# TritonDataCenter/containerpilot

Hardware: AMD Instinct MI355X
Metric: events/sec (higher is better)
Workload: dtype n/a (CPU daemon, no tensor math; see BASELINE.json north_star); 1 GPU; model=containerpilot daemon, BASELINE stress shape scaled to 550 jobs, jobs=550, watches=50, parallelism=1 independent daemons (1/rank)

## Files before the change

### containerpilot_amd/native.py

```python

import ctypes
import json
import os

from . import REPO_ROOT

_LIB_PATH = os.path.join(REPO_ROOT, "containerpilot_amd", "_native.so")
_lib = None


def _load():
    global _lib
    if _lib is None:
        if not os.path.exists(_LIB_PATH):
            raise RuntimeError(
                "native library missing: %s (run __graft_entry__.build())"
                % _LIB_PATH)
        _lib = ctypes.CDLL(_LIB_PATH)
        _lib.cp_version.restype = ctypes.c_char_p
        _lib.cp_render_template.restype = ctypes.c_void_p
        _lib.cp_render_template.argtypes = [
            ctypes.c_char_p, ctypes.POINTER(ctypes.c_void_p)]
        _lib.cp_parse_duration_ns.restype = ctypes.c_longlong
        _lib.cp_parse_duration_ns.argtypes = [ctypes.c_char_p]
# ... 11 lines not shown
        _lib.cp_validate_config.argtypes = [ctypes.c_char_p]
        _lib.cp_consul_endpoint.restype = ctypes.c_void_p
        _lib.cp_consul_endpoint.argtypes = [
            ctypes.c_char_p, ctypes.POINTER(ctypes.c_void_p)]
        _lib.cp_watch_render.restype = ctypes.c_void_p
        _lib.cp_watch_render.argtypes = [
            ctypes.c_char_p, ctypes.c_char_p, ctypes.c_char_p,
            ctypes.c_char_p, ctypes.c_char_p,
            ctypes.POINTER(ctypes.c_void_p)]
        _lib.cp_kv_decode.restype = ctypes.c_void_p
        _lib.cp_kv_decode.argtypes = [
            ctypes.c_char_p, ctypes.c_size_t,
            ctypes.POINTER(ctypes.c_void_p)]
        _lib.cp_kv_render.restype = ctypes.c_void_p
        _lib.cp_kv_render.argtypes = [
            ctypes.c_char_p, ctypes.c_char_p, ctypes.c_size_t,
            ctypes.c_char_p, ctypes.c_char_p, ctypes.c_int,
            ctypes.c_char_p, ctypes.POINTER(ctypes.c_size_t),
            ctypes.POINTER(ctypes.c_void_p)]
        _lib.cp_sensor_extract.restype = ctypes.c_int
        _lib.cp_sensor_extract.argtypes = [
            ctypes.c_char_p, ctypes.c_size_t, ctypes.c_char_p,
            ctypes.POINTER(ctypes.c_double),
            ctypes.POINTER(ctypes.c_void_p)]
        _lib.cp_signal_number.restype = ctypes.c_int
        _lib.cp_signal_number.argtypes = [
            ctypes.c_char_p, ctypes.POINTER(ctypes.c_void_p)]
        _lib.cp_metrics_replay.restype = ctypes.c_void_p
        _lib.cp_metrics_replay.argtypes = [
            ctypes.c_char_p, ctypes.POINTER(ctypes.c_void_p)]
        _lib.cp_metric_value_string.restype = ctypes.c_void_p
        _lib.cp_metric_value_string.argtypes = [
            ctypes.c_char_p, ctypes.POINTER(ctypes.c_void_p)]
        _lib.cp_free.argtypes = [ctypes.c_void_p]
    return _lib


def _take_string(lib, ptr):
    if not ptr:
        return None
    out = ctypes.string_at(ptr).decode()
    lib.cp_free(ptr)
    return out


def version():
    return _load().cp_version().decode()


def render_template(text):
    lib = _load()
    err = ctypes.c_void_p()
    out = lib.cp_render_template(text.encode(), ctypes.byref(err))
    if not out:
        raise ValueError(_take_string(lib, err.value))
    return _take_string(lib, out)


def parse_duration_ns(text):
    ns = _load().cp_parse_duration_ns(text.encode())
    if ns < 0:
        raise ValueError("invalid duration: %s" % text)
    return ns


def parse_duration(text):
# ... 77 lines not shown
    err = ctypes.c_void_p()
    out = lib.cp_kv_decode(body, len(body), ctypes.byref(err))
    if not out:
        raise ValueError(_take_string(lib, err.value))
    return json.loads(_take_string(lib, out))


def kv_render(template_text, body, name, key, prefix=False, dc=""):
    lib = _load()
    if isinstance(body, str):
        body = body.encode()
    err = ctypes.c_void_p()
    size = ctypes.c_size_t()
    out = lib.cp_kv_render(template_text.encode(), body,
                           len(body) if body is not None else 0,
                           name.encode(), key.encode(), int(bool(prefix)),
                           dc.encode(), ctypes.byref(size), ctypes.byref(err))
    if not out:
        raise ValueError(_take_string(lib, err.value))
    rendered = ctypes.string_at(out, size.value)
    lib.cp_free(out)
    return rendered


def metrics_replay(script_json):
    lib = _load()
    err = ctypes.c_void_p()
    out = lib.cp_metrics_replay(script_json.encode(), ctypes.byref(err))
    if not out:
        raise ValueError(_take_string(lib, err.value))
    return _take_string(lib, out)


def metric_value_string(json_text):
    lib = _load()
    err = ctypes.c_void_p()
    out = lib.cp_metric_value_string(json_text.encode(), ctypes.byref(err))
    if not out:
        raise ValueError(_take_string(lib, err.value))
    return _take_string(lib, out)
```

### cpp/include/cpilot/command.hpp

```cpp
#pragma once

#include <memory>
#include <string>
#include <vector>

#include "cpilot/events.hpp"
#include "cpilot/json.hpp"
#include "cpilot/loop.hpp"
#include "cpilot/timing.hpp"

namespace cpilot {

bool parseArgs(const Json& raw, std::string* exec,
               std::vector<std::string>* args, std::string* err);

class Command : public std::enable_shared_from_this<Command> {
 public:
  Command(std::string execPath, std::vector<std::string> args, Duration timeout,
          bool raw, std::string logField);
  Command(const Command&) = delete;
  Command& operator=(const Command&) = delete;

  const std::string& name() const { return name_; }
  void setName(std::string name) { name_ = std::move(name); }
  const std::string& execPath() const { return exec_; }

  std::string envName() const;

  void run(Loop& loop, std::shared_ptr<Bus> bus);

  void term();
  void kill();

  bool running() const { return running_; }
  pid_t pid() const { return pid_; }

 private:
  void spawn(Loop& loop, std::shared_ptr<Bus> bus);
  void onExit(Loop& loop, std::shared_ptr<Bus> bus, int status);

  std::string name_;
  std::string exec_;
  std::vector<std::string> args_;
  Duration timeout_;
  bool raw_;
  std::string logField_;
  std::string pidEnvName_;

  pid_t pid_ = -1;
  bool running_ = false;
  bool pendingRun_ = false;
  int pendingSignal_ = 0;
  Loop* loop_ = nullptr;
  uint64_t timeoutTimer_ = 0;
  TimePoint tReq_{}, tCb_{};
  int logFd_ = -1;
  std::string logBuf_;
};

using CommandPtr = std::shared_ptr<Command>;

void commandEnvInvalidate();

CommandPtr newCommand(const Json& rawExec, Duration timeout, bool raw,
                      const std::string& logField, std::string* err);

}
```

### cpp/include/cpilot/spawner.hpp

```cpp
#pragma once

#include <sys/types.h>

#include <cstdint>
#include <deque>
#include <functional>
#include <map>
#include <memory>
#include <mutex>
#include <string>
#include <thread>
#include <vector>

#include "cpilot/loop.hpp"

namespace cpilot {

class Spawner {
 public:
  using SpawnCb = std::function<void(pid_t pid, int err)>;

  static Spawner& global();

  void spawn(Loop& loop, const std::string& execPath,
             const std::vector<std::string>& args,
             std::shared_ptr<const std::vector<std::string>> baseEnv,
             const std::vector<std::string>& extraEnv, int stdioFd,
             SpawnCb cb);

  int helperCount() const { return (int)helpers_.size(); }

  size_t backlog();
  bool overloaded();

 private:
  Spawner();
  struct Helper {
    int sock = -1;
    pid_t pid = -1;
    bool dead = false;
    std::deque<std::pair<std::vector<char>, int>> overflow;
    std::mutex sendMu;
  };
  struct Pending {
    Loop* loop;
    uint64_t loopId;
    SpawnCb cb;
    size_t helperIdx;
  };

  bool launchHelper(Helper* h);
  void flushOverflow(size_t idx);
  void readerMain();
  void handleMessage(size_t idx, const char* buf, size_t len);
  void helperDied(size_t idx);
  bool sendRequest(Helper& h, const std::vector<char>& buf, int fd);
  void wakeReader();

  std::string helperPath_;
  std::vector<std::unique_ptr<Helper>> helpers_;
  size_t nextHelper_ = 0;

  std::mutex mu_;
  std::map<uint32_t, Pending> pending_;
  uint32_t nextReqId_ = 1;
  std::map<pid_t, std::pair<Loop*, uint64_t>> pidLoops_;

  int wakeFds_[2] = {-1, -1};
  std::thread reader_;
};

}
```

### cpp/include/cpilot/spawnproto.hpp

```cpp
#pragma once

#include <cstdint>

namespace cpilot {
namespace spawnproto {

constexpr int kHelperFd = 3;

enum MsgType : uint32_t {
  kSpawnRequest = 1,
  kSpawnReply = 2,
  kChildExit = 3,
};

struct RequestHeader {
  uint32_t type;
  uint32_t reqId;
  uint32_t argc;
  uint32_t envc;
  uint8_t wantStdio;
  uint8_t pad[3];
};

struct Reply {
  uint32_t type;
  uint32_t reqId;
  int32_t pid;
  int32_t err;
};

struct ExitNotice {
  uint32_t type;
  uint32_t pad;
  int32_t pid;
  int32_t status;
};

constexpr size_t kMaxRequestBytes = 1024 * 1024;

}
}
```

### cpp/src/command.cpp

```cpp
#include "cpilot/command.hpp"

#include <fcntl.h>
#include <signal.h>
#include <sys/epoll.h>
#include <sys/wait.h>
#include <unistd.h>

#include <cctype>
#include <cstring>
#include <cstdio>
#include <map>

#include "cpilot/log.hpp"
#include "cpilot/spawner.hpp"

extern char** environ;

namespace cpilot {

namespace {

std::map<std::string, std::string>& pidEnvOverlay() {
  static std::map<std::string, std::string> overlay;
  return overlay;
}

std::shared_ptr<const std::vector<std::string>>& baseEnvCache() {
  static std::shared_ptr<const std::vector<std::string>> cache;
  return cache;
}
bool& baseEnvDirty() {
  static bool dirty = true;
  return dirty;
}

std::shared_ptr<const std::vector<std::string>> baseEnvSnapshot() {
  if (!baseEnvDirty() && baseEnvCache()) return baseEnvCache();
// ... 20 lines not shown

const std::vector<std::string>& overlayExtras() { return overlayStrings(); }

void overlaySet(const std::string& key, const std::string& value) {
  auto [it, inserted] = pidEnvOverlay().emplace(key, value);
  if (inserted) {
    overlayIndex()[key] = overlayStrings().size();
    overlayStrings().push_back(key + "=" + value);
    if (getenv(key.c_str())) baseEnvDirty() = true;
  } else {
    it->second = value;
    overlayStrings()[overlayIndex()[key]] = key + "=" + value;
  }
}

void overlayErase(const std::string& key) {
  if (pidEnvOverlay().erase(key)) {
    auto idxIt = overlayIndex().find(key);
    if (idxIt != overlayIndex().end()) {
      size_t slot = idxIt->second;
      overlayIndex().erase(idxIt);
      auto& strs = overlayStrings();
      if (slot + 1 != strs.size()) {
        strs[slot] = std::move(strs.back());
        size_t eq = strs[slot].find('=');
        overlayIndex()[strs[slot].substr(0, eq)] = slot;
      }
      strs.pop_back();
    }
    if (getenv(key.c_str())) baseEnvDirty() = true;
  }
}

}

void commandEnvInvalidate() { baseEnvDirty() = true; }

bool parseArgs(const Json& raw, std::string* execPath,
               std::vector<std::string>* args, std::string* err) {
  std::vector<std::string> all;
  if (raw.isString()) {
    std::string s = raw.str();
    size_t a = 0, b = s.size();
    while (a < b && isspace((unsigned char)s[a])) a++;
    while (b > a && isspace((unsigned char)s[b - 1])) b--;
    s = s.substr(a, b - a);
    if (!s.empty()) {
      std::string cur;
      for (char c : s) {
        if (c == ' ') {
          all.push_back(cur);
          cur.clear();
        } else {
          cur += c;
        }
      }
      all.push_back(cur);
    }
  } else if (raw.isArray()) {
    for (auto& e : raw.array()) {
      if (e.isString()) all.push_back(e.str());
      else all.push_back(e.dump());
    }
  } else if (!raw.isNull()) {
    *err = "unable to parse exec arguments";
    return false;
  }
  if (all.empty()) {
    *err = "received zero-length argument";
// ... 8 lines not shown
                      const std::string& logField, std::string* err) {
  std::string execPath;
  std::vector<std::string> args;
  if (!parseArgs(rawExec, &execPath, &args, err)) return nullptr;
  return std::make_shared<Command>(execPath, args, timeout, raw, logField);
}

Command::Command(std::string execPath, std::vector<std::string> args,
                 Duration timeout, bool raw, std::string logField)
    : name_(execPath),
      exec_(std::move(execPath)),
      args_(std::move(args)),
      timeout_(timeout),
      raw_(raw),
      logField_(std::move(logField)) {}

std::string Command::envName() const {
  if (name_.empty()) return name_;
  std::string name = name_;
  size_t slash = name.find_last_of('/');
  if (slash != std::string::npos) name = name.substr(slash + 1);
  size_t dot = name.find_last_of('.');
  if (dot != std::string::npos && dot > 0)
    name = name.substr(0, dot) + name.substr(name.size());
  std::string out;
  for (char c : name) {
    if (isalnum((unsigned char)c)) {
      out += (char)toupper((unsigned char)c);
    } else if (out.empty() || out.back() != '_') {
      out += '_';
    }
  }
  return out;
}

void Command::run(Loop& loop, std::shared_ptr<Bus> bus) {
  if (running_) {
    LOG_DEBUG("%s already running, queueing run", name_.c_str());
    pendingRun_ = true;
    return;
  }
  spawn(loop, std::move(bus));
}

void Command::spawn(Loop& loop, std::shared_ptr<Bus> bus) {
  loop_ = &loop;
  LOG_DEBUG("%s.Run start", name_.c_str());

  int pipefds[2] = {-1, -1};
  if (!raw_) {
    if (pipe2(pipefds, O_CLOEXEC) != 0) {
      LOG_ERROR("unable to create pipe for %s: %s", name_.c_str(),
                strerror(errno));
      bus->publish(Event{EventCode::ExitFailed, name_});
      bus->publish(Event{EventCode::Error, strerror(errno)});
      return;
    }
  }

  running_ = true;
  pid_ = -1;
  pendingSignal_ = 0;
  tReq_ = Clock::now();
  auto self = shared_from_this();
  int readFd = pipefds[0];
  auto baseEnv = baseEnvSnapshot();
// ... 37 lines not shown
                  logBuf_.clear();
                }
                loop_->unwatchFd(logFd_);
                close(logFd_);
                logFd_ = -1;
                return;
              } else {
                return;
              }
            }
          });
        }

        if (timeout_ > Duration(0)) {
          timeoutTimer_ = loop_->addTimeout(timeout_, [this, self] {
            LOG_WARN("%s timeout after %llds", name_.c_str(),
                     (long long)std::chrono::duration_cast<
                         std::chrono::seconds>(timeout_)
                         .count());
            timeoutTimer_ = 0;
            kill();
          });
        }

        if (pendingSignal_ != 0) {
          ::kill(-pid, pendingSignal_);
          pendingSignal_ = 0;
        }

        loop_->watchChild(pid, [this, self, bus](int status) {
          onExit(*loop_, bus, status);
        });
      };
  Spawner::global().spawn(loop, exec_, args_, std::move(baseEnv),
                          overlayExtras(), raw_ ? -1 : pipefds[1],
                          std::move(compCb));
}

void Command::onExit(Loop& loop, std::shared_ptr<Bus> bus, int status) {
  LOG_DEBUG("%s.Run end", name_.c_str());
  static const bool rttDebug = cpilotDebugEnv("CPILOT_LOOP_DEBUG");
  if (rttDebug) {
    auto now = Clock::now();
    double total =
        std::chrono::duration<double, std::milli>(now - tReq_).count();
    if (total > 50.0) {
      double execPhase =
          std::chrono::duration<double, std::milli>(now - tCb_).count();
      fprintf(stderr,
              "spawn rtt: %s total=%.0fms spawn_phase=%.0fms "
              "exec_phase=%.0fms\n",
              name_.c_str(), total, total - execPhase, execPhase);
    }
  }
  if (timeoutTimer_) {
    loop.cancelTimer(timeoutTimer_);
    timeoutTimer_ = 0;
  }
  if (logFd_ >= 0) {
    char buf[4096];
    ssize_t n;
    while ((n = read(logFd_, buf, sizeof(buf))) > 0) logBuf_.append(buf, n);
    size_t pos;
    while ((pos = logBuf_.find('\n')) != std::string::npos) {
      logging::logFields(logging::Level::Info, logField_, pid_,
                         logBuf_.substr(0, pos));
      logBuf_.erase(0, pos + 1);
// ... 56 lines not shown
```

### cpp/src/pyapi.cpp

```cpp
#include <cstdlib>
#include <cstring>
#include <map>
#include <stdexcept>
#include <string>
#include <vector>

#include "cpilot/config.hpp"
#include "cpilot/control.hpp"
#include "cpilot/discovery.hpp"
#include "cpilot/json.hpp"
#include "cpilot/sensor.hpp"
#include "cpilot/signals.hpp"
#include "cpilot/telemetry.hpp"
#include "cpilot/timing.hpp"
#include "cpilot/tmpl.hpp"
#include "cpilot/version.hpp"
#include "cpilot/watches.hpp"

using namespace cpilot;

namespace {
char* dupString(const std::string& s) {
  char* out = (char*)malloc(s.size() + 1);
  memcpy(out, s.c_str(), s.size() + 1);
  return out;
}
}

extern "C" {

const char* cp_version() { return kVersion; }

void cp_free(char* p) { free(p); }

char* cp_render_template(const char* text, char** errOut) {
  try {
    return dupString(renderTemplate(text));
  } catch (const std::exception& e) {
    if (errOut) *errOut = dupString(e.what());
    return nullptr;
  }
}

char* cp_render_data(const char* templateText, const char* dataJson,
                     char** errOut) {
// ... 130 lines not shown
}

int cp_sensor_extract(const char* body, size_t bodyLen, const char* recordJson,
                      double* out, char** errOut) {
  try {
    sensor::RecordSpec rec;
    std::string key, err;
    if (!sensor::parseRecord(parseJson5(recordJson), &rec, &key, &err)) {
      if (errOut)
        *errOut = dupString("record" + key + (key.empty() ? ": " : " ") + err);
      return 0;
    }
    double value = 0;
    if (!sensor::extract(std::string(body, bodyLen), rec, &value, &err)) {
      if (errOut) *errOut = dupString(err);
      return 0;
    }
    if (out) *out = value;
    return 1;
  } catch (const std::exception& e) {
    if (errOut) *errOut = dupString(e.what());
    return 0;
  }
}

int cp_signal_number(const char* name, char** errOut) {
  int signo = 0;
  if (signals::fromName(name, &signo, nullptr)) return signo;
  if (errOut)
    *errOut = dupString(std::string("'") + name +
                        "' is not accepted: must be one of " +
                        signals::acceptedNames());
  return -1;
}

char* cp_metrics_replay(const char* scriptJson, char** errOut) {
  try {
    Json script = parseJson5(scriptJson);
    prom::Registry registry;
    std::string err;
    std::vector<std::shared_ptr<MetricConfig>> cfgs;
    if (const Json* m = script.find("metrics")) {
      if (!newMetricConfigs(*m, &cfgs, &err, &registry)) {
        if (errOut) *errOut = dupString(err);
        return nullptr;
      }
    }
    std::vector<std::shared_ptr<Metric>> metrics;
    for (auto& cfg : cfgs) metrics.push_back(std::make_shared<Metric>(cfg));
    if (const Json* events = script.find("events")) {
      for (auto& e : events->array())
        for (auto& metric : metrics)
          metric->onEvent(Event{EventCode::Metric, e.str()});
    }

    auto need = [](const Json& obj, const char* key) -> const Json& {
      const Json* v = obj.find(key);
      if (!v) throw std::runtime_error(std::string("script: missing ") + key);
      return *v;
    };
    auto strings = [](const Json* v) {
      std::vector<std::string> out;
      if (v)
        for (auto& s : v->array()) out.push_back(s.str());
      return out;
    };
// ... 59 lines not shown
```

### cpp/src/spawner.cpp

```cpp
#include "cpilot/spawner.hpp"

#include <fcntl.h>
#include <limits.h>
#include <poll.h>
#include <signal.h>
#include <spawn.h>
#include <string.h>
#include <sys/socket.h>
#include <unistd.h>

#include <cstdio>
#include <cstdlib>

#include "cpilot/log.hpp"
#include "cpilot/spawnproto.hpp"

extern char** environ;

namespace cpilot {

using namespace spawnproto;

namespace {

int defaultHelperCount() {
  if (const char* v = getenv("CPILOT_SPAWN_HELPERS")) {
    int n = atoi(v);
    if (n >= 1 && n <= 64) return n;
  }
  long ncpu = sysconf(_SC_NPROCESSORS_ONLN);
  if (ncpu < 1) ncpu = 1;
  int n = (int)(ncpu / 16);
  if (n < 2) n = 2;
  if (n > 8) n = 8;
  return n;
}

std::string findHelperBinary() {
  if (const char* v = getenv("CPILOT_SPAWN_HELPER")) return v;
  char buf[PATH_MAX];
  ssize_t n = readlink("/proc/self/exe", buf, sizeof(buf) - 1);
  if (n > 0) {
    buf[n] = 0;
    std::string dir(buf);
    size_t slash = dir.find_last_of('/');
    if (slash != std::string::npos) {
      std::string candidate = dir.substr(0, slash) + "/cpilot-spawn-helper";
      if (access(candidate.c_str(), X_OK) == 0) return candidate;
    }
  }
  return "cpilot-spawn-helper";
}

bool spawnDebug() {
  static bool on = cpilotDebugEnv("CPILOT_SPAWN_DEBUG");
  return on;
}

}

Spawner& Spawner::global() {
  static Spawner* s = new Spawner();
  return *s;
}

Spawner::Spawner() {
  helperPath_ = findHelperBinary();
  if (pipe2(wakeFds_, O_NONBLOCK | O_CLOEXEC) != 0)
    LOG_ERROR("spawner: pipe2 failed: %s", strerror(errno));
  int n = defaultHelperCount();
  for (int i = 0; i < n; i++) helpers_.push_back(std::make_unique<Helper>());
  for (auto& h : helpers_) {
    if (!launchHelper(h.get())) {
      logging::logf(logging::Level::Fatal,
                    "spawner: cannot launch spawn helper '%s': %s",
                    helperPath_.c_str(), strerror(errno));
    }
  }
  reader_ = std::thread([this] { readerMain(); });
  reader_.detach();
}

bool Spawner::launchHelper(Helper* h) {
  int socks[2];
  if (socketpair(AF_UNIX, SOCK_SEQPACKET | SOCK_CLOEXEC, 0, socks) != 0)
    return false;
  int bufsz = 1 << 20;
  setsockopt(socks[0], SOL_SOCKET, SO_SNDBUF, &bufsz, sizeof(bufsz));
  setsockopt(socks[1], SOL_SOCKET, SO_SNDBUF, &bufsz, sizeof(bufsz));
  fcntl(socks[0], F_SETFL, O_NONBLOCK);

  posix_spawn_file_actions_t actions;
  posix_spawn_file_actions_init(&actions);
  posix_spawn_file_actions_adddup2(&actions, socks[1], kHelperFd);
  posix_spawnattr_t attr;
  posix_spawnattr_init(&attr);
  sigset_t empty;
  sigemptyset(&empty);
  posix_spawnattr_setsigmask(&attr, &empty);
  posix_spawnattr_setflags(&attr, POSIX_SPAWN_SETSIGMASK);

  char* argv[] = {const_cast<char*>("cpilot-spawn-helper"), nullptr};
  pid_t pid = -1;
  int rc = posix_spawn(&pid, helperPath_.c_str(), &actions, &attr, argv,
                       environ);
  posix_spawn_file_actions_destroy(&actions);
  posix_spawnattr_destroy(&attr);
  close(socks[1]);
  if (rc != 0) {
    close(socks[0]);
    errno = rc;
    return false;
  }
  h->sock = socks[0];
  h->pid = pid;
  h->dead = false;
  return true;
}

size_t Spawner::backlog() {
  std::lock_guard<std::mutex> l(mu_);
  return pending_.size();
}

void Spawner::flushOverflow(size_t idx) {
  Helper& h = *helpers_[idx];
  while (true) {
    std::deque<std::pair<std::vector<char>, int>> batch;
    {
      std::lock_guard<std::mutex> l(mu_);
      if (h.dead || h.overflow.empty()) return;
      for (int i = 0; i < 16 && !h.overflow.empty(); i++) {
        batch.push_back(std::move(h.overflow.front()));
        h.overflow.pop_front();
      }
    }
    size_t sent = 0;
    {
      std::lock_guard<std::mutex> sl(h.sendMu);
      for (auto& [buf, fd] : batch) {
        if (!sendRequest(h, buf, fd)) break;
        if (fd >= 0) close(fd);
        sent++;
      }
    }
    if (sent < batch.size()) {
      std::lock_guard<std::mutex> l(mu_);
      for (size_t i = batch.size(); i > sent; i--)
        h.overflow.push_front(std::move(batch[i - 1]));
      return;
    }
  }
}

bool Spawner::overloaded() {
  return backlog() > helpers_.size() * 16;
}

void Spawner::wakeReader() {
  char b = 1;
  ssize_t unused = write(wakeFds_[1], &b, 1);
  (void)unused;
}

void Spawner::spawn(Loop& loop, const std::string& execPath,
                    const std::vector<std::string>& args,
                    std::shared_ptr<const std::vector<std::string>> baseEnv,
                    const std::vector<std::string>& extraEnv, int stdioFd,
                    SpawnCb cb) {
  RequestHeader hdr;
  memset(&hdr, 0, sizeof(hdr));
  hdr.type = kSpawnRequest;
  hdr.argc = 1 + (uint32_t)args.size();
  hdr.envc = (uint32_t)((baseEnv ? baseEnv->size() : 0) + extraEnv.size());
  hdr.wantStdio = stdioFd >= 0 ? 1 : 0;

  size_t size = sizeof(hdr) + execPath.size() + 1;
  for (auto& a : args) size += a.size() + 1;
  if (baseEnv)
    for (auto& e : *baseEnv) size += e.size() + 1;
  for (auto& e : extraEnv) size += e.size() + 1;
  if (size > kMaxRequestBytes) {
    if (stdioFd >= 0) close(stdioFd);
    loop.post([cb] { cb(-1, E2BIG); });
    return;
  }

  std::vector<char> buf;
  buf.reserve(size);
  auto append = [&buf](const std::string& s) {
    buf.insert(buf.end(), s.begin(), s.end());
    buf.push_back('\0');
  };
  buf.resize(sizeof(hdr));
  append(execPath);
  for (auto& a : args) append(a);
  if (baseEnv)
    for (auto& e : *baseEnv) append(e);
  for (auto& e : extraEnv) append(e);

  size_t idx = 0;
  uint32_t reqId = 0;
  bool queued = false;
  {
    std::lock_guard<std::mutex> l(mu_);
    reqId = nextReqId_++;
    hdr.reqId = reqId;
    memcpy(buf.data(), &hdr, sizeof(hdr));

    bool found = false;
    for (size_t i = 0; i < helpers_.size(); i++) {
      idx = (nextHelper_ + i) % helpers_.size();
      if (!helpers_[idx]->dead) {
        found = true;
        break;
      }
    }
    nextHelper_ = (idx + 1) % helpers_.size();
    if (!found) {
      if (stdioFd >= 0) close(stdioFd);
      loop.post([cb] { cb(-1, ECHILD); });
      return;
    }
    pending_[reqId] = Pending{&loop, loop.id(), std::move(cb), idx};
    if (!helpers_[idx]->overflow.empty()) {
      helpers_[idx]->overflow.emplace_back(std::move(buf), stdioFd);
      queued = true;
    }
  }
  if (spawnDebug())
    fprintf(stderr, "[spawner] req %u -> helper %zu\n", reqId, idx);
  if (queued) {
    wakeReader();
    return;
  }
  Helper& h = *helpers_[idx];
  bool sent;
  {
    std::lock_guard<std::mutex> sl(h.sendMu);
    sent = sendRequest(h, buf, stdioFd);
  }
  if (!sent) {
    std::lock_guard<std::mutex> l(mu_);
    h.overflow.emplace_back(std::move(buf), stdioFd);
    wakeReader();
    return;
  }
  if (stdioFd >= 0) close(stdioFd);
}

bool Spawner::sendRequest(Helper& h, const std::vector<char>& buf, int fd) {
  struct iovec iov{const_cast<char*>(buf.data()), buf.size()};
  struct msghdr msg;
  memset(&msg, 0, sizeof(msg));
  msg.msg_iov = &iov;
  msg.msg_iovlen = 1;
  char cmsgBuf[CMSG_SPACE(sizeof(int))];
  if (fd >= 0) {
    memset(cmsgBuf, 0, sizeof(cmsgBuf));
    msg.msg_control = cmsgBuf;
    msg.msg_controllen = sizeof(cmsgBuf);
    struct cmsghdr* c = CMSG_FIRSTHDR(&msg);
    c->cmsg_level = SOL_SOCKET;
    c->cmsg_type = SCM_RIGHTS;
    c->cmsg_len = CMSG_LEN(sizeof(int));
    memcpy(CMSG_DATA(c), &fd, sizeof(int));
  }
  while (true) {
    ssize_t n = sendmsg(h.sock, &msg, MSG_NOSIGNAL);
    if (spawnDebug())
      fprintf(stderr, "[spawner] sendmsg fd=%d n=%zd errno=%d\n", h.sock, n,
              n < 0 ? errno : 0);
    if (n >= 0) return true;
    if (errno == EINTR) continue;
    return false;
  }
}

void Spawner::readerMain() {
  resetThreadScheduling();
  std::vector<char> buf(64);
  while (true) {
    std::vector<struct pollfd> fds;
    {
      std::lock_guard<std::mutex> l(mu_);
      for (auto& h : helpers_) {
        short ev = h->dead ? 0 : POLLIN;
        if (!h->dead && !h->overflow.empty()) ev |= POLLOUT;
        fds.push_back({h->sock, ev, 0});
      }
    }
    fds.push_back({wakeFds_[0], POLLIN, 0});
    int rc = poll(fds.data(), (nfds_t)fds.size(), 1000);
    if (spawnDebug() && rc != 0) {
      fprintf(stderr, "[spawner] poll rc=%d", rc);
      for (size_t i = 0; i < fds.size(); i++)
        fprintf(stderr, " fd%d=%x", fds[i].fd, fds[i].revents);
      fprintf(stderr, "\n");
    }
    if (rc < 0) {
      if (errno == EINTR) continue;
      return;
    }
    if (fds.back().revents & POLLIN) {
      char drain[256];
      while (read(wakeFds_[0], drain, sizeof(drain)) > 0) {
      }
    }
    for (size_t i = 0; i + 1 < fds.size(); i++) {
      if (fds[i].revents & POLLOUT) flushOverflow(i);
      if (fds[i].revents & (POLLIN | POLLHUP | POLLERR)) {
        while (true) {
          ssize_t n = recv(fds[i].fd, buf.data(), buf.size(), MSG_DONTWAIT);
          if (n > 0) {
// ... 4 lines not shown
          }
          if (n < 0 && (errno == EAGAIN || errno == EINTR)) break;
          if (spawnDebug())
            fprintf(stderr, "[spawner] helper %zu died n=%zd errno=%d\n",
                    i, n, errno);
          helperDied(i);
          break;
        }
      }
    }
  }
}

void Spawner::handleMessage(size_t idx, const char* data, size_t len) {
  uint32_t type = 0;
  if (len >= sizeof(uint32_t)) memcpy(&type, data, sizeof(type));
  if (spawnDebug() && type != kSpawnReply && type != kChildExit)
    fprintf(stderr, "[spawner] DROP unknown msg type=%u len=%zu\n", type, len);
  if (type == kSpawnReply && len >= sizeof(Reply)) {
    Reply r;
    memcpy(&r, data, sizeof(r));
    Pending p;
    {
      std::lock_guard<std::mutex> l(mu_);
      auto it = pending_.find(r.reqId);
      if (it == pending_.end()) {
        if (spawnDebug())
          fprintf(stderr, "[spawner] DROP reply for unknown req %u\n",
                  r.reqId);
        return;
      }
      p = std::move(it->second);
      pending_.erase(it);
    }
    if (spawnDebug())
      fprintf(stderr, "[spawner] reply req %u pid %d\n", r.reqId, r.pid);
    if (r.pid > 0) pidLoops_[r.pid] = {p.loop, p.loopId};
    SpawnCb cb = std::move(p.cb);
    pid_t pid = r.pid;
    int err = r.err;
    Loop::postIfLive(p.loop, p.loopId,
                     timedItem("spawncb", [cb, pid, err] { cb(pid, err); }));
  } else if (type == kChildExit && len >= sizeof(ExitNotice)) {
    ExitNotice note;
    memcpy(&note, data, sizeof(note));
    auto it = pidLoops_.find(note.pid);
    if (it == pidLoops_.end()) {
      if (spawnDebug())
        fprintf(stderr, "[spawner] DROP exit notice for unknown pid %d\n",
                note.pid);
      return;
    }
    if (spawnDebug())
      fprintf(stderr, "[spawner] exit pid %d\n", note.pid);
    auto [loop, loopId] = it->second;
    pidLoops_.erase(it);
    pid_t pid = note.pid;
    int status = note.status;
    Loop::postIfLive(loop, loopId, timedItem("exit", [loop, pid, status] {
                       loop->notifyChildExit(pid, status);
                     }));
  }
}

void Spawner::helperDied(size_t idx) {
  std::vector<Pending> lost;
  {
    std::lock_guard<std::mutex> l(mu_);
    Helper& h = *helpers_[idx];
    if (h.dead) return;
    h.dead = true;
    LOG_ERROR("spawner: helper %d (pid %d) died; respawning",
              (int)idx, (int)h.pid);
    for (auto it = pending_.begin(); it != pending_.end();) {
      if (it->second.helperIdx == idx) {
        lost.push_back(std::move(it->second));
        it = pending_.erase(it);
      } else {
        ++it;
      }
    }
    for (auto& [obuf, ofd] : h.overflow)
      if (ofd >= 0) close(ofd);
    h.overflow.clear();
    close(h.sock);
    if (!launchHelper(&h)) {
      LOG_ERROR("spawner: helper respawn failed: %s", strerror(errno));
      h.dead = true;
    }
  }
  for (auto& p : lost) {
    SpawnCb cb = std::move(p.cb);
    Loop::postIfLive(p.loop, p.loopId, [cb] { cb(-1, ECHILD); });
  }
// ... 4 lines not shown
```

### cpp/src/spawnhelper_main.cpp

```cpp
#include <errno.h>
#include <fcntl.h>
#include <poll.h>
#include <signal.h>
#include <sched.h>
#include <spawn.h>
#include <sys/resource.h>
#include <stdio.h>
#include <stdlib.h>
#include <string.h>
#include <sys/socket.h>
#include <sys/wait.h>
#include <unistd.h>

#include <vector>

#include "cpilot/spawnproto.hpp"

using namespace cpilot::spawnproto;

namespace {

int selfPipe[2] = {-1, -1};

bool helperDebug() {
  const char* v = getenv("CPILOT_SPAWN_DEBUG");
  static bool on = v && v[0] && !(v[0] == '0' && !v[1]);
  return on;
}

void onSigchld(int) {
  char b = 1;
  ssize_t unused = write(selfPipe[1], &b, 1);
  (void)unused;
}

bool sendAll(int fd, const void* buf, size_t len) {
  while (true) {
    ssize_t n = send(fd, buf, len, MSG_NOSIGNAL);
    if (n == (ssize_t)len) return true;
    if (n < 0 && (errno == EINTR)) continue;
    if (n < 0 && errno == EAGAIN) {
      struct pollfd p{fd, POLLOUT, 0};
      poll(&p, 1, 1000);
      continue;
    }
    return false;
  }
}

void reapAndNotify(int sock) {
  while (true) {
    int status = 0;
    pid_t pid = waitpid(-1, &status, WNOHANG);
    if (pid <= 0) return;
    if (helperDebug())
      fprintf(stderr, "[helper %d] reaped pid %d\n", getpid(), (int)pid);
    ExitNotice note{kChildExit, 0, (int32_t)pid, (int32_t)status};
    if (!sendAll(sock, &note, sizeof(note))) _exit(0);
  }
}

void handleRequest(int sock, const char* buf, size_t len, int stdioFd) {
  if (len < sizeof(RequestHeader)) return;
  RequestHeader hdr;
  memcpy(&hdr, buf, sizeof(hdr));
  const char* p = buf + sizeof(hdr);
  const char* end = buf + len;

  std::vector<const char*> argv, envp;
  for (uint32_t i = 0; i < hdr.argc + hdr.envc && p < end; i++) {
    if (i < hdr.argc)
      argv.push_back(p);
    else
      envp.push_back(p);
    p += strnlen(p, end - p) + 1;
  }
  Reply reply{kSpawnReply, hdr.reqId, -1, EINVAL};
  if (argv.size() == hdr.argc && envp.size() == hdr.envc && !argv.empty()) {
    argv.push_back(nullptr);
    envp.push_back(nullptr);

    posix_spawnattr_t attr;
    posix_spawnattr_init(&attr);
    sigset_t empty;
    sigemptyset(&empty);
    posix_spawnattr_setsigmask(&attr, &empty);
    posix_spawnattr_setpgroup(&attr, 0);
    short flags = POSIX_SPAWN_SETPGROUP | POSIX_SPAWN_SETSIGMASK;
#ifdef POSIX_SPAWN_USEVFORK
    flags |= POSIX_SPAWN_USEVFORK;
#endif
    posix_spawnattr_setflags(&attr, flags);

    posix_spawn_file_actions_t actions;
    posix_spawn_file_actions_init(&actions);
    if (hdr.wantStdio && stdioFd >= 0) {
      posix_spawn_file_actions_adddup2(&actions, stdioFd, 1);
      posix_spawn_file_actions_adddup2(&actions, stdioFd, 2);
    }
    pid_t pid = -1;
    int rc = posix_spawnp(&pid, argv[0], &actions, &attr,
                          const_cast<char**>(argv.data()),
                          const_cast<char**>(envp.data()));
    posix_spawn_file_actions_destroy(&actions);
    posix_spawnattr_destroy(&attr);
    reply.pid = (rc == 0) ? (int32_t)pid : -1;
    reply.err = rc;
    if (helperDebug())
      fprintf(stderr, "[helper %d] spawned pid %d req %u\n", getpid(),
              (int)pid, hdr.reqId);
  }
  if (stdioFd >= 0) close(stdioFd);
  if (!sendAll(sock, &reply, sizeof(reply))) _exit(0);
}

}

int cpilotSpawnHelperMain() {
  {
    struct sched_param sp;
    memset(&sp, 0, sizeof(sp));
    sched_setscheduler(0, SCHED_OTHER, &sp);
    setpriority(PRIO_PROCESS, 0, 0);
  }
  const int sock = kHelperFd;
  fcntl(sock, F_SETFD, FD_CLOEXEC);
  if (pipe2(selfPipe, O_NONBLOCK | O_CLOEXEC) != 0) _exit(1);

  struct sigaction sa;
  memset(&sa, 0, sizeof(sa));
  sa.sa_handler = onSigchld;
  sa.sa_flags = SA_RESTART | SA_NOCLDSTOP;
  sigaction(SIGCHLD, &sa, nullptr);
  signal(SIGPIPE, SIG_IGN);
  sigset_t none;
  sigemptyset(&none);
  sigprocmask(SIG_SETMASK, &none, nullptr);

  std::vector<char> buf(kMaxRequestBytes);
  char cmsgBuf[CMSG_SPACE(sizeof(int))];

  while (true) {
    struct pollfd fds[2] = {{sock, POLLIN, 0}, {selfPipe[0], POLLIN, 0}};
    int rc = poll(fds, 2, -1);
    if (helperDebug())
      fprintf(stderr, "[helper %d] poll rc=%d sock=%x pipe=%x\n", getpid(),
              rc, fds[0].revents, fds[1].revents);
    if (rc < 0) {
      if (errno == EINTR) {
        reapAndNotify(sock);
        continue;
      }
      _exit(1);
    }
    if (fds[1].revents & POLLIN) {
      char drain[256];
      while (read(selfPipe[0], drain, sizeof(drain)) > 0) {
      }
      reapAndNotify(sock);
    }
    if (fds[0].revents & (POLLIN | POLLHUP | POLLERR)) {
      struct iovec iov{buf.data(), buf.size()};
      struct msghdr msg;
      memset(&msg, 0, sizeof(msg));
      msg.msg_iov = &iov;
      msg.msg_iovlen = 1;
      msg.msg_control = cmsgBuf;
      msg.msg_controllen = sizeof(cmsgBuf);
      ssize_t n = recvmsg(sock, &msg, MSG_CMSG_CLOEXEC);
      if (helperDebug())
        fprintf(stderr, "[helper %d] recvmsg n=%zd errno=%d\n", getpid(), n,
                n < 0 ? errno : 0);
      if (n == 0) _exit(0);
      if (n < 0) {
        if (errno == EINTR || errno == EAGAIN) continue;
        _exit(0);
      }
      int passedFd = -1;
      for (struct cmsghdr* c = CMSG_FIRSTHDR(&msg); c;
           c = CMSG_NXTHDR(&msg, c)) {
        if (c->cmsg_level == SOL_SOCKET && c->cmsg_type == SCM_RIGHTS)
          memcpy(&passedFd, CMSG_DATA(c), sizeof(int));
      }
      handleRequest(sock, buf.data(), (size_t)n, passedFd);
      reapAndNotify(sock);
    }
  }
}

#ifndef CPILOT_HELPER_NO_MAIN
int main() { return cpilotSpawnHelperMain(); }
#endif
```

Baseline: 11000 events/s.

## Rework spawn helpers: cgroup-aware sizing, load-balanced dispatch, batched exits, cached exec paths

```diff
diff --git a/containerpilot_amd/native.py b/containerpilot_amd/native.py
--- a/containerpilot_amd/native.py
+++ b/containerpilot_amd/native.py
@@ -67,6 +67,12 @@
         _lib.cp_metric_value_string.restype = ctypes.c_void_p
         _lib.cp_metric_value_string.argtypes = [
             ctypes.c_char_p, ctypes.POINTER(ctypes.c_void_p)]
+        _lib.cp_spawn_helper_count.restype = ctypes.c_int
+        _lib.cp_spawn_helper_count.argtypes = [
+            ctypes.c_long, ctypes.c_long, ctypes.c_char_p, ctypes.c_char_p]
+        _lib.cp_resolve_executable.restype = ctypes.c_void_p
+        _lib.cp_resolve_executable.argtypes = [
+            ctypes.c_char_p, ctypes.c_char_p, ctypes.POINTER(ctypes.c_int)]
         _lib.cp_free.argtypes = [ctypes.c_void_p]
     return _lib
 
@@ -210,6 +216,25 @@
     return _take_string(lib, out)
 
 
+def spawn_helper_count(online_cpus, affinity_cpus, cpu_max=None,
+                       env_override=None):
+    return _load().cp_spawn_helper_count(
+        online_cpus, affinity_cpus,
+        None if cpu_max is None else cpu_max.encode(),
+        None if env_override is None else env_override.encode())
+
+
+def resolve_executable(name, path_value):
+    lib = _load()
+    err = ctypes.c_int()
+    out = lib.cp_resolve_executable(
+        name.encode(), None if path_value is None else path_value.encode(),
+        ctypes.byref(err))
+    if not out:
+        raise OSError(err.value, os.strerror(err.value), name)
+    return _take_string(lib, out)
+
+
 def metric_value_string(json_text):
     lib = _load()
     err = ctypes.c_void_p()
diff --git a/cpp/include/cpilot/command.hpp b/cpp/include/cpilot/command.hpp
--- a/cpp/include/cpilot/command.hpp
+++ b/cpp/include/cpilot/command.hpp
@@ -13,6 +13,9 @@
 
 bool parseArgs(const Json& raw, std::string* exec,
                std::vector<std::string>* args, std::string* err);
+
+int resolveExecutable(const std::string& name, const char* pathValue,
+                      std::string* file);
 
 class Command : public std::enable_shared_from_this<Command> {
  public:
@@ -38,9 +41,14 @@
  private:
   void spawn(Loop& loop, std::shared_ptr<Bus> bus);
   void onExit(Loop& loop, std::shared_ptr<Bus> bus, int status);
+  const std::string& resolvedFile();
 
   std::string name_;
   std::string exec_;
+  std::string file_;
+  std::string filePath_;
+  bool filePathSet_ = false;
+  uint64_t fileEnvGen_ = 0;
   std::vector<std::string> args_;
   Duration timeout_;
   bool raw_;
diff --git a/cpp/include/cpilot/spawner.hpp b/cpp/include/cpilot/spawner.hpp
--- a/cpp/include/cpilot/spawner.hpp
+++ b/cpp/include/cpilot/spawner.hpp
@@ -16,13 +16,19 @@
 
 namespace cpilot {
 
+constexpr int kCpusPerSpawnHelper = 3;
+constexpr int kMinSpawnHelpers = 2;
+constexpr int kMaxSpawnHelpers = 8;
+int spawnHelperCount(long onlineCpus, long affinityCpus, const char* cpuMax,
+                     const char* envOverride);
+
 class Spawner {
  public:
   using SpawnCb = std::function<void(pid_t pid, int err)>;
 
   static Spawner& global();
 
-  void spawn(Loop& loop, const std::string& execPath,
+  void spawn(Loop& loop, const std::string& execPath, const std::string& file,
              const std::vector<std::string>& args,
              std::shared_ptr<const std::vector<std::string>> baseEnv,
              const std::vector<std::string>& extraEnv, int stdioFd,
@@ -39,6 +45,7 @@
     int sock = -1;
     pid_t pid = -1;
     bool dead = false;
+    size_t outstanding = 0;
     std::deque<std::pair<std::vector<char>, int>> overflow;
     std::mutex sendMu;
   };
@@ -60,6 +67,7 @@
   std::string helperPath_;
   std::vector<std::unique_ptr<Helper>> helpers_;
   size_t nextHelper_ = 0;
+  size_t shedDepth_;
 
   std::mutex mu_;
   std::map<uint32_t, Pending> pending_;
diff --git a/cpp/include/cpilot/spawnproto.hpp b/cpp/include/cpilot/spawnproto.hpp
--- a/cpp/include/cpilot/spawnproto.hpp
+++ b/cpp/include/cpilot/spawnproto.hpp
@@ -19,7 +19,8 @@
   uint32_t argc;
   uint32_t envc;
   uint8_t wantStdio;
-  uint8_t pad[3];
+  uint8_t hasFile;
+  uint8_t pad[2];
 };
 
 struct Reply {
@@ -36,6 +37,8 @@
   int32_t status;
 };
 
+constexpr size_t kMaxExitBatch = 32;
+
 constexpr size_t kMaxRequestBytes = 1024 * 1024;
 
 }
diff --git a/cpp/src/command.cpp b/cpp/src/command.cpp
--- a/cpp/src/command.cpp
+++ b/cpp/src/command.cpp
@@ -3,6 +3,7 @@
 #include <fcntl.h>
 #include <signal.h>
 #include <sys/epoll.h>
+#include <sys/stat.h>
 #include <sys/wait.h>
 #include <unistd.h>
 
@@ -89,9 +90,46 @@
   }
 }
 
-}
-
-void commandEnvInvalidate() { baseEnvDirty() = true; }
+uint64_t& envGeneration() {
+  static uint64_t gen = 1;
+  return gen;
+}
+
+}
+
+void commandEnvInvalidate() {
+  baseEnvDirty() = true;
+  envGeneration()++;
+}
+
+int resolveExecutable(const std::string& name, const char* pathValue,
+                      std::string* file) {
+  if (name.empty()) return ENOENT;
+  if (name.find('/') != std::string::npos) {
+    *file = name;
+    return 0;
+  }
+  const char* p = pathValue ? pathValue : "/bin:/usr/bin";
+  bool sawEacces = false;
+  while (true) {
+    const char* colon = strchr(p, ':');
+    size_t len = colon ? (size_t)(colon - p) : strlen(p);
+    std::string candidate = len ? std::string(p, len) + "/" + name : name;
+    struct stat st;
+    if (stat(candidate.c_str(), &st) == 0) {
+      if (S_ISREG(st.st_mode) && access(candidate.c_str(), X_OK) == 0) {
+        *file = candidate;
+        return 0;
+      }
+      sawEacces = true;
+    } else if (errno == EACCES) {
+      sawEacces = true;
+    }
+    if (!colon) break;
+    p = colon + 1;
+  }
+  return sawEacces ? EACCES : ENOENT;
+}
 
 bool parseArgs(const Json& raw, std::string* execPath,
                std::vector<std::string>* args, std::string* err) {
@@ -166,6 +204,22 @@
     }
   }
   return out;
+}
+
+const std::string& Command::resolvedFile() {
+  const char* path = getenv("PATH");
+  bool fresh = !file_.empty() && fileEnvGen_ == envGeneration() &&
+               filePathSet_ == (path != nullptr) &&
+               (!path || filePath_ == path);
+  if (!fresh) {
+    file_.clear();
+    if (resolveExecutable(exec_, path, &file_) == 0) {
+      fileEnvGen_ = envGeneration();
+      filePathSet_ = path != nullptr;
+      filePath_ = path ? path : "";
+    }
+  }
+  return file_;
 }
 
 void Command::run(Loop& loop, std::shared_ptr<Bus> bus) {
@@ -269,7 +323,8 @@
           onExit(*loop_, bus, status);
         });
       };
-  Spawner::global().spawn(loop, exec_, args_, std::move(baseEnv),
+  Spawner::global().spawn(loop, exec_, resolvedFile(), args_,
+                          std::move(baseEnv),
                           overlayExtras(), raw_ ? -1 : pipefds[1],
                           std::move(compCb));
 }
diff --git a/cpp/src/pyapi.cpp b/cpp/src/pyapi.cpp
--- a/cpp/src/pyapi.cpp
+++ b/cpp/src/pyapi.cpp
@@ -5,12 +5,14 @@
 #include <string>
 #include <vector>
 
+#include "cpilot/command.hpp"
 #include "cpilot/config.hpp"
 #include "cpilot/control.hpp"
 #include "cpilot/discovery.hpp"
 #include "cpilot/json.hpp"
 #include "cpilot/sensor.hpp"
 #include "cpilot/signals.hpp"
+#include "cpilot/spawner.hpp"
 #include "cpilot/telemetry.hpp"
 #include "cpilot/timing.hpp"
 #include "cpilot/tmpl.hpp"
@@ -207,6 +209,19 @@
                         "' is not accepted: must be one of " +
                         signals::acceptedNames());
   return -1;
+}
+
+int cp_spawn_helper_count(long onlineCpus, long affinityCpus,
+                          const char* cpuMax, const char* envOverride) {
+  return spawnHelperCount(onlineCpus, affinityCpus, cpuMax, envOverride);
+}
+
+char* cp_resolve_executable(const char* name, const char* pathValue,
+                            int* errnoOut) {
+  std::string file;
+  int rc = resolveExecutable(name, pathValue, &file);
+  if (errnoOut) *errnoOut = rc;
+  return rc == 0 ? dupString(file) : nullptr;
 }
 
 char* cp_metrics_replay(const char* scriptJson, char** errOut) {
diff --git a/cpp/src/spawner.cpp b/cpp/src/spawner.cpp
--- a/cpp/src/spawner.cpp
+++ b/cpp/src/spawner.cpp
@@ -3,6 +3,7 @@
 #include <fcntl.h>
 #include <limits.h>
 #include <poll.h>
+#include <sched.h>
 #include <signal.h>
 #include <spawn.h>
 #include <string.h>
@@ -23,17 +24,64 @@
 
 namespace {
 
+double cpuMaxQuota(const char* text) {
+  if (!text) return 0;
+  double quota = 0, period = 0;
+  if (sscanf(text, "%lf %lf", &quota, &period) != 2) return 0;
+  if (quota <= 0 || period <= 0) return 0;
+  return quota / period;
+}
+
+std::string readCpuMax() {
+  std::string group;
+  if (FILE* f = fopen("/proc/self/cgroup", "r")) {
+    char line[PATH_MAX + 16];
+    while (fgets(line, sizeof(line), f)) {
+      if (strncmp(line, "0::", 3) != 0) continue;
+      group = line + 3;
+      while (!group.empty() && (group.back() == '\n' || group.back() == '/'))
+        group.pop_back();
+      break;
+    }
+    fclose(f);
+  }
+  std::string best;
+  double bestQuota = 0;
+  while (true) {
+    std::string path = "/sys/fs/cgroup" + group + "/cpu.max";
+    if (FILE* f = fopen(path.c_str(), "r")) {
+      char text[128];
+      if (fgets(text, sizeof(text), f)) {
+        double q = cpuMaxQuota(text);
+        if (q > 0 && (bestQuota == 0 || q < bestQuota)) {
+          bestQuota = q;
+          best = text;
+        }
+      }
+      fclose(f);
+    }
+    if (group.empty()) break;
+    size_t slash = group.find_last_of('/');
+    group.erase(slash == std::string::npos ? 0 : slash);
+  }
+  return best;
+}
+
 int defaultHelperCount() {
-  if (const char* v = getenv("CPILOT_SPAWN_HELPERS")) {
+  long affinity = 0;
+  cpu_set_t set;
+  if (sched_getaffinity(0, sizeof(set), &set) == 0) affinity = CPU_COUNT(&set);
+  std::string cpuMax = readCpuMax();
+  return spawnHelperCount(sysconf(_SC_NPROCESSORS_ONLN), affinity,
+                          cpuMax.c_str(), getenv("CPILOT_SPAWN_HELPERS"));
+}
+
+size_t shedDepth() {
+  if (const char* v = getenv("CPILOT_SPAWN_SHED_DEPTH")) {
     int n = atoi(v);
-    if (n >= 1 && n <= 64) return n;
-  }
-  long ncpu = sysconf(_SC_NPROCESSORS_ONLN);
-  if (ncpu < 1) ncpu = 1;
-  int n = (int)(ncpu / 16);
-  if (n < 2) n = 2;
-  if (n > 8) n = 8;
-  return n;
+    if (n >= 1 && n <= 1024) return (size_t)n;
+  }
+  return 16;
 }
 
 std::string findHelperBinary() {
@@ -59,6 +107,26 @@
 
 }
 
+int spawnHelperCount(long onlineCpus, long affinityCpus, const char* cpuMax,
+                     const char* envOverride) {
+  if (envOverride) {
+    int n = atoi(envOverride);
+    if (n >= 1 && n <= 64) return n;
+  }
+  double budget = 0;
+  auto take = [&budget](double cpus) {
+    if (cpus >= 1 && (budget == 0 || cpus < budget)) budget = cpus;
+  };
+  take((double)onlineCpus);
+  take((double)affinityCpus);
+  double quota = cpuMaxQuota(cpuMax);
+  if (quota > 0) take(quota < 1 ? 1 : quota);
+  int n = (int)(budget / kCpusPerSpawnHelper);
+  if (n < kMinSpawnHelpers) n = kMinSpawnHelpers;
+  if (n > kMaxSpawnHelpers) n = kMaxSpawnHelpers;
+  return n;
+}
+
 Spawner& Spawner::global() {
   static Spawner* s = new Spawner();
   return *s;
@@ -68,6 +136,7 @@
   helperPath_ = findHelperBinary();
   if (pipe2(wakeFds_, O_NONBLOCK | O_CLOEXEC) != 0)
     LOG_ERROR("spawner: pipe2 failed: %s", strerror(errno));
+  shedDepth_ = shedDepth();
   int n = defaultHelperCount();
   for (int i = 0; i < n; i++) helpers_.push_back(std::make_unique<Helper>());
   for (auto& h : helpers_) {
@@ -115,6 +184,7 @@
   h->sock = socks[0];
   h->pid = pid;
   h->dead = false;
+  h->outstanding = 0;
   return true;
 }
 
@@ -154,7 +224,15 @@
 }
 
 bool Spawner::overloaded() {
-  return backlog() > helpers_.size() * 16;
+  std::lock_guard<std::mutex> l(mu_);
+  bool live = false;
+  size_t least = 0;
+  for (auto& h : helpers_) {
+    if (h->dead) continue;
+    if (!live || h->outstanding < least) least = h->outstanding;
+    live = true;
+  }
+  return live && least > shedDepth_;
 }
 
 void Spawner::wakeReader() {
@@ -164,6 +242,7 @@
 }
 
 void Spawner::spawn(Loop& loop, const std::string& execPath,
+                    const std::string& file,
                     const std::vector<std::string>& args,
                     std::shared_ptr<const std::vector<std::string>> baseEnv,
                     const std::vector<std::string>& extraEnv, int stdioFd,
@@ -174,8 +253,10 @@
   hdr.argc = 1 + (uint32_t)args.size();
   hdr.envc = (uint32_t)((baseEnv ? baseEnv->size() : 0) + extraEnv.size());
   hdr.wantStdio = stdioFd >= 0 ? 1 : 0;
+  hdr.hasFile = file.empty() ? 0 : 1;
 
   size_t size = sizeof(hdr) + execPath.size() + 1;
+  if (hdr.hasFile) size += file.size() + 1;
   for (auto& a : args) size += a.size() + 1;
   if (baseEnv)
     for (auto& e : *baseEnv) size += e.size() + 1;
@@ -193,6 +274,7 @@
     buf.push_back('\0');
   };
   buf.resize(sizeof(hdr));
+  if (hdr.hasFile) append(file);
   append(execPath);
   for (auto& a : args) append(a);
   if (baseEnv)
@@ -210,18 +292,21 @@
 
     bool found = false;
     for (size_t i = 0; i < helpers_.size(); i++) {
-      idx = (nextHelper_ + i) % helpers_.size();
-      if (!helpers_[idx]->dead) {
+      size_t cand = (nextHelper_ + i) % helpers_.size();
+      if (helpers_[cand]->dead) continue;
+      if (!found ||
+          helpers_[cand]->outstanding < helpers_[idx]->outstanding) {
+        idx = cand;
         found = true;
-        break;
-      }
-    }
-    nextHelper_ = (idx + 1) % helpers_.size();
+      }
+    }
     if (!found) {
       if (stdioFd >= 0) close(stdioFd);
       loop.post([cb] { cb(-1, ECHILD); });
       return;
     }
+    nextHelper_ = (idx + 1) % helpers_.size();
+    helpers_[idx]->outstanding++;
     pending_[reqId] = Pending{&loop, loop.id(), std::move(cb), idx};
     if (!helpers_[idx]->overflow.empty()) {
       helpers_[idx]->overflow.emplace_back(std::move(buf), stdioFd);
@@ -279,7 +364,7 @@
 
 void Spawner::readerMain() {
   resetThreadScheduling();
-  std::vector<char> buf(64);
+  std::vector<char> buf(kMaxExitBatch * sizeof(ExitNotice));
   while (true) {
     std::vector<struct pollfd> fds;
     {
@@ -350,6 +435,8 @@
       }
       p = std::move(it->second);
       pending_.erase(it);
+      if (p.helperIdx == idx && helpers_[idx]->outstanding > 0)
+        helpers_[idx]->outstanding--;
     }
     if (spawnDebug())
       fprintf(stderr, "[spawner] reply req %u pid %d\n", r.reqId, r.pid);
@@ -359,25 +446,29 @@
     int err = r.err;
     Loop::postIfLive(p.loop, p.loopId,
                      timedItem("spawncb", [cb, pid, err] { cb(pid, err); }));
-  } else if (type == kChildExit && len >= sizeof(ExitNotice)) {
-    ExitNotice note;
-    memcpy(&note, data, sizeof(note));
-    auto it = pidLoops_.find(note.pid);
-    if (it == pidLoops_.end()) {
+  } else if (type == kChildExit) {
+    for (size_t off = 0; off + sizeof(ExitNotice) <= len;
+         off += sizeof(ExitNotice)) {
+      ExitNotice note;
+      memcpy(&note, data + off, sizeof(note));
+      if (note.type != kChildExit) break;
+      auto it = pidLoops_.find(note.pid);
+      if (it == pidLoops_.end()) {
+        if (spawnDebug())
+          fprintf(stderr, "[spawner] DROP exit notice for unknown pid %d\n",
+                  note.pid);
+        continue;
+      }
       if (spawnDebug())
-        fprintf(stderr, "[spawner] DROP exit notice for unknown pid %d\n",
-                note.pid);
-      return;
-    }
-    if (spawnDebug())
-      fprintf(stderr, "[spawner] exit pid %d\n", note.pid);
-    auto [loop, loopId] = it->second;
-    pidLoops_.erase(it);
-    pid_t pid = note.pid;
-    int status = note.status;
-    Loop::postIfLive(loop, loopId, timedItem("exit", [loop, pid, status] {
-                       loop->notifyChildExit(pid, status);
-                     }));
+        fprintf(stderr, "[spawner] exit pid %d\n", note.pid);
+      auto [loop, loopId] = it->second;
+      pidLoops_.erase(it);
+      pid_t pid = note.pid;
+      int status = note.status;
+      Loop::postIfLive(loop, loopId, timedItem("exit", [loop, pid, status] {
+                         loop->notifyChildExit(pid, status);
+                       }));
+    }
   }
 }
 
diff --git a/cpp/src/spawnhelper_main.cpp b/cpp/src/spawnhelper_main.cpp
--- a/cpp/src/spawnhelper_main.cpp
+++ b/cpp/src/spawnhelper_main.cpp
@@ -8,6 +8,7 @@
 #include <stdio.h>
 #include <stdlib.h>
 #include <string.h>
+#include <sys/signalfd.h>
 #include <sys/socket.h>
 #include <sys/wait.h>
 #include <unistd.h>
@@ -20,18 +21,12 @@
 
 namespace {
 
-int selfPipe[2] = {-1, -1};
+constexpr int kRequestsPerPass = 8;
 
 bool helperDebug() {
   const char* v = getenv("CPILOT_SPAWN_DEBUG");
   static bool on = v && v[0] && !(v[0] == '0' && !v[1]);
   return on;
-}
-
-void onSigchld(int) {
-  char b = 1;
-  ssize_t unused = write(selfPipe[1], &b, 1);
-  (void)unused;
 }
 
 bool sendAll(int fd, const void* buf, size_t len) {
@@ -49,14 +44,20 @@
 }
 
 void reapAndNotify(int sock) {
+  ExitNotice notes[kMaxExitBatch];
   while (true) {
-    int status = 0;
-    pid_t pid = waitpid(-1, &status, WNOHANG);
-    if (pid <= 0) return;
-    if (helperDebug())
-      fprintf(stderr, "[helper %d] reaped pid %d\n", getpid(), (int)pid);
-    ExitNotice note{kChildExit, 0, (int32_t)pid, (int32_t)status};
-    if (!sendAll(sock, &note, sizeof(note))) _exit(0);
+    size_t n = 0;
+    while (n < kMaxExitBatch) {
+      int status = 0;
+      pid_t pid = waitpid(-1, &status, WNOHANG);
+      if (pid <= 0) break;
+      if (helperDebug())
+        fprintf(stderr, "[helper %d] reaped pid %d\n", getpid(), (int)pid);
+      notes[n++] = ExitNotice{kChildExit, 0, (int32_t)pid, (int32_t)status};
+    }
+    if (n == 0) return;
+    if (!sendAll(sock, notes, n * sizeof(ExitNotice))) _exit(0);
+    if (n < kMaxExitBatch) return;
   }
 }
 
@@ -67,6 +68,11 @@
   const char* p = buf + sizeof(hdr);
   const char* end = buf + len;
 
+  const char* file = nullptr;
+  if (hdr.hasFile && p < end) {
+    file = p;
+    p += strnlen(p, end - p) + 1;
+  }
   std::vector<const char*> argv, envp;
   for (uint32_t i = 0; i < hdr.argc + hdr.envc && p < end; i++) {
     if (i < hdr.argc)
@@ -76,7 +82,8 @@
     p += strnlen(p, end - p) + 1;
   }
   Reply reply{kSpawnReply, hdr.reqId, -1, EINVAL};
-  if (argv.size() == hdr.argc && envp.size() == hdr.envc && !argv.empty()) {
+  if (argv.size() == hdr.argc && envp.size() == hdr.envc && !argv.empty() &&
+      (!hdr.hasFile || file) && end[-1] == '\0') {
     argv.push_back(nullptr);
     envp.push_back(nullptr);
 
@@ -99,9 +106,15 @@
       posix_spawn_file_actions_adddup2(&actions, stdioFd, 2);
     }
     pid_t pid = -1;
-    int rc = posix_spawnp(&pid, argv[0], &actions, &attr,
-                          const_cast<char**>(argv.data()),
-                          const_cast<char**>(envp.data()));
+    int rc = ENOENT;
+    if (file)
+      rc = posix_spawn(&pid, file, &actions, &attr,
+                       const_cast<char**>(argv.data()),
+                       const_cast<char**>(envp.data()));
+    if (!file || rc == ENOENT || rc == EACCES || rc == ENOEXEC)
+      rc = posix_spawnp(&pid, argv[0], &actions, &attr,
+                        const_cast<char**>(argv.data()),
+                        const_cast<char**>(envp.data()));
     posix_spawn_file_actions_destroy(&actions);
     posix_spawnattr_destroy(&attr);
     reply.pid = (rc == 0) ? (int32_t)pid : -1;
@@ -125,65 +138,63 @@
   }
   const int sock = kHelperFd;
   fcntl(sock, F_SETFD, FD_CLOEXEC);
-  if (pipe2(selfPipe, O_NONBLOCK | O_CLOEXEC) != 0) _exit(1);
-
-  struct sigaction sa;
-  memset(&sa, 0, sizeof(sa));
-  sa.sa_handler = onSigchld;
-  sa.sa_flags = SA_RESTART | SA_NOCLDSTOP;
-  sigaction(SIGCHLD, &sa, nullptr);
+
   signal(SIGPIPE, SIG_IGN);
-  sigset_t none;
-  sigemptyset(&none);
-  sigprocmask(SIG_SETMASK, &none, nullptr);
+  signal(SIGCHLD, SIG_DFL);
+  sigset_t chld;
+  sigemptyset(&chld);
+  sigaddset(&chld, SIGCHLD);
+  sigprocmask(SIG_SETMASK, &chld, nullptr);
+  const int sigFd = signalfd(-1, &chld, SFD_NONBLOCK | SFD_CLOEXEC);
+  if (sigFd < 0) _exit(1);
 
   std::vector<char> buf(kMaxRequestBytes);
   char cmsgBuf[CMSG_SPACE(sizeof(int))];
 
   while (true) {
-    struct pollfd fds[2] = {{sock, POLLIN, 0}, {selfPipe[0], POLLIN, 0}};
+    struct pollfd fds[2] = {{sock, POLLIN, 0}, {sigFd, POLLIN, 0}};
     int rc = poll(fds, 2, -1);
     if (helperDebug())
-      fprintf(stderr, "[helper %d] poll rc=%d sock=%x pipe=%x\n", getpid(),
+      fprintf(stderr, "[helper %d] poll rc=%d sock=%x sig=%x\n", getpid(),
               rc, fds[0].revents, fds[1].revents);
     if (rc < 0) {
-      if (errno == EINTR) {
+      if (errno == EINTR) continue;
+      _exit(1);
+    }
+    if (fds[1].revents & POLLIN) {
+      struct signalfd_siginfo si;
+      ssize_t unused = read(sigFd, &si, sizeof(si));
+      (void)unused;
+      reapAndNotify(sock);
+    }
+    if (fds[0].revents & (POLLIN | POLLHUP | POLLERR | POLLNVAL)) {
+      for (int taken = 0; taken < kRequestsPerPass; taken++) {
+        struct iovec iov{buf.data(), buf.size()};
+        struct msghdr msg;
+        memset(&msg, 0, sizeof(msg));
+        msg.msg_iov = &iov;
+        msg.msg_iovlen = 1;
+        msg.msg_control = cmsgBuf;
+        msg.msg_controllen = sizeof(cmsgBuf);
+        ssize_t n = recvmsg(sock, &msg, MSG_CMSG_CLOEXEC | MSG_DONTWAIT);
+        if (helperDebug())
+          fprintf(stderr, "[helper %d] recvmsg n=%zd errno=%d\n", getpid(), n,
+                  n < 0 ? errno : 0);
+        if (n == 0) _exit(0);
+        if (n < 0) {
+          if (errno == EINTR) continue;
+          if (errno == EAGAIN) break;
+          _exit(0);
+        }
+        int passedFd = -1;
+        for (struct cmsghdr* c = CMSG_FIRSTHDR(&msg); c;
+             c = CMSG_NXTHDR(&msg, c)) {
+          if (c->cmsg_level == SOL_SOCKET && c->cmsg_type == SCM_RIGHTS)
+            memcpy(&passedFd, CMSG_DATA(c), sizeof(int));
+        }
+        handleRequest(sock, buf.data(), (size_t)n, passedFd);
         reapAndNotify(sock);
-        continue;
       }
-      _exit(1);
-    }
-    if (fds[1].revents & POLLIN) {
-      char drain[256];
-      while (read(selfPipe[0], drain, sizeof(drain)) > 0) {
-      }
-      reapAndNotify(sock);
-    }
-    if (fds[0].revents & (POLLIN | POLLHUP | POLLERR)) {
-      struct iovec iov{buf.data(), buf.size()};
-      struct msghdr msg;
-      memset(&msg, 0, sizeof(msg));
-      msg.msg_iov = &iov;
-      msg.msg_iovlen = 1;
-      msg.msg_control = cmsgBuf;
-      msg.msg_controllen = sizeof(cmsgBuf);
-      ssize_t n = recvmsg(sock, &msg, MSG_CMSG_CLOEXEC);
-      if (helperDebug())
-        fprintf(stderr, "[helper %d] recvmsg n=%zd errno=%d\n", getpid(), n,
-                n < 0 ? errno : 0);
-      if (n == 0) _exit(0);
-      if (n < 0) {
-        if (errno == EINTR || errno == EAGAIN) continue;
-        _exit(0);
-      }
-      int passedFd = -1;
-      for (struct cmsghdr* c = CMSG_FIRSTHDR(&msg); c;
-           c = CMSG_NXTHDR(&msg, c)) {
-        if (c->cmsg_level == SOL_SOCKET && c->cmsg_type == SCM_RIGHTS)
-          memcpy(&passedFd, CMSG_DATA(c), sizeof(int));
-      }
-      handleRequest(sock, buf.data(), (size_t)n, passedFd);
-      reapAndNotify(sock);
     }
   }
 }
```

Measured after the change: 10990 events/s. No clear change (-0.2%).
